# XuZerui2023/Radar-Signal-Process

Hardware: AMD Instinct MI355X
Metric: CPIs/sec (4096 range × 128 pulse) through PC→MTD→CFAR; achieved HBM GB/s (higher is better)
Workload: dtype f32

## Files before the change

include/rsp.h:

```cpp
#ifndef RSP_H
#define RSP_H

#include <stddef.h>
#include <stdint.h>

#ifdef __cplusplus
extern "C" {
#endif

#define RSP_ABI_VERSION 5
#define RSP_MAX_SEG 4
#define RSP_MAX_FIR_TAPS 64

typedef struct rsp_ctx rsp_ctx;

typedef enum {
    RSP_OK = 0,
    RSP_ERR_ARG = 1,
    RSP_ERR_SHAPE = 2,
    RSP_ERR_UNSUPPORTED = 3,
    RSP_ERR_CFAR_WINDOW = 4,
    RSP_ERR_HIP = 5,
    RSP_ERR_NOMEM = 6
} rsp_status;
// ... 98 lines not shown
int rsp_pc_mtd_cfar_f64(rsp_ctx* ctx, const void* echo, int32_t dtype, int32_t layout,
                        int64_t P, int64_t R, int64_t batch, const rsp_cfar_params* cfar,
                        double* rdm_out , int32_t out_layout, double* flag_out,
                        double* flagV_out );
int rsp_cfar_f64(rsp_ctx* ctx, const double* rdm, int32_t rdm_layout, int64_t V, int64_t R,
                 int64_t batch, const rsp_cfar_params* cfar, double* flag_out,
                 double* flagV_out );

int rsp_pc_mtd_cfar_dev(rsp_ctx* ctx, const void* d_echo, int32_t dtype, int64_t batch,
                        const rsp_cfar_params* cfar, float* d_rdm, uint8_t* d_flag,
                        uint8_t* d_flagV, void* stream);

int rsp_cfar_dev(rsp_ctx* ctx, const float* d_rdm, int64_t V, int64_t R, int64_t batch,
                 const rsp_cfar_params* cfar, uint8_t* d_flag, uint8_t* d_flagV,
                 void* stream);

int rsp_mtd_cfar_dev(rsp_ctx* ctx, const void* d_pc, int64_t batch, const rsp_cfar_params* cfar,
                     float* d_rdm, uint8_t* d_flag, uint8_t* d_flagV, void* stream);

int rsp_pc_mtd_cfar_diff_dev(rsp_ctx* ctx, const void* d_echo, int32_t dtype, int64_t batch,
                             const rsp_cfar_params* cfar, float* d_sum, float* d_diff,
                             uint8_t* d_flag, uint8_t* d_flagV, void* stream);

int rsp_window_pc_mtd_cfar_dev(rsp_ctx* ctx, const void* d_frames, int32_t dtype, int64_t beams,
                               int64_t frames, int32_t win, const rsp_cfar_params* cfar,
                               float* d_rdm, uint8_t* d_flag, uint8_t* d_flagV, void* stream);

int rsp_pc_dev(rsp_ctx* ctx, const void* d_echo, int32_t dtype, int64_t batch, void* d_pc,
               void* stream);

int rsp_set_pc_split(rsp_ctx* ctx, int32_t enable);

int rsp_set_pc_prune(rsp_ctx* ctx, int32_t enable);

typedef struct {
    int32_t nfft;
    int32_t nsub;
    int32_t sub_step;
    int32_t zin;
    int32_t zout;
    int32_t fir;
} rsp_pc_plan_seg;
typedef struct {
    int32_t specialised;
    int32_t fused;
    int32_t prune;
    int32_t nmf;
    rsp_pc_plan_seg seg[RSP_MAX_SEG];
} rsp_pc_plan_t;
int rsp_pc_plan(rsp_ctx* ctx, rsp_pc_plan_t* out, int32_t n);

enum { RSP_CFAR_R_COPY = 0,
       RSP_CFAR_R_GENERIC = 1,
       RSP_CFAR_R_4CELL = 2,
       RSP_CFAR_R_16CELL = 3 };
enum { RSP_RANGE_NONE = 0,
       RSP_RANGE_GROUPED = 1,
       RSP_RANGE_JOB57 = 2,
       RSP_RANGE_PREV_HITS = 3,
       RSP_RANGE_PER_CHUNK = 4 };
enum { RSP_HITS_NONE = 0,
       RSP_HITS_BATCHED57 = 1,
       RSP_HITS_PER_HIT57 = 2,
       RSP_HITS_PER_HIT_RUNTIME = 3 };
typedef struct {
    int32_t fused;
// ... 231 lines not shown
```

radar-signal-process_amd/csrc/rsp_capi.cpp:

```cpp
#include <hip/hip_runtime.h>

#include <cmath>
#include <complex>
#include <cstdarg>
#include <cstdio>
#include <cstdlib>
#include <cstring>
#include <map>
#include <new>
#include <string>
#include <vector>

#include "rsp_ctx.h"

using rsp::make_window;
using rsp::scratch_acquire;
using rsp::scratch_release;
using rsp::upload;

using cd = std::complex<double>;

static thread_local std::string g_err;

int fail(rsp_ctx* ctx, int code, const char* fmt, ...) {
    char buf[512];
    va_list ap;
    va_start(ap, fmt);
    vsnprintf(buf, sizeof(buf), fmt, ap);
    va_end(ap);
    if (ctx) ctx->err = buf;
    g_err = buf;
    return code;
}


static double mround(double x) { return x >= 0 ? std::floor(x + 0.5) : -std::floor(-x + 0.5); }

static double bessel_i0(double x) {
    double sum = 1.0, term = 1.0, q = x * x / 4.0;
    for (int k = 1; k < 500; ++k) {
        term *= q / ((double)k * k);
        sum += term;
        if (term < 1e-18 * sum) break;
    }
    return sum;
}
// ... 741 lines not shown
    if (!ctx) return fail(nullptr, RSP_ERR_ARG, "rsp_set_range_concat: null ctx");
    if (ctx->cfar_only) return fail(ctx, RSP_ERR_ARG, "rsp_set_range_concat: CFAR-only context");
    if (nparts < 0 || nparts > RSP_MAX_SEG || (nparts > 0 && (!src_start || !len)))
        return fail(ctx, RSP_ERR_ARG, "rsp_set_range_concat: bad part list (%d parts)", nparts);
    int64_t w = 0;
    for (int i = 0; i < nparts; ++i) {
        if (len[i] < 1 || src_start[i] < 0 || src_start[i] + len[i] > ctx->pc_w)
            return fail(ctx, RSP_ERR_ARG, "rsp_set_range_concat: part %d [%lld, +%lld) outside the %lld PC columns", i,
                        (long long)src_start[i], (long long)len[i], (long long)ctx->pc_w);
        w += len[i];
    }
    if (!set_device(ctx)) return fail(ctx, RSP_ERR_HIP, "hipSetDevice failed");
    HIP_TRY(ctx, hipDeviceSynchronize());
    ctx->ncat = nparts;
    for (int i = 0; i < nparts; ++i) {
        ctx->cat_src[i] = src_start[i];
        ctx->cat_len[i] = len[i];
    }
    ctx->p.R_out = nparts > 0 ? w : ctx->pc_w;
    ctx->mtd.R_out = (int)ctx->p.R_out;
    return RSP_OK;
}

static bool pc_fused(const rsp_ctx* ctx) {
    return ctx->pc_mf.size() == 2 && rsp::pc_pair_supported(ctx->pc_mf[0].mf.nfft, ctx->pc_mf[1].mf.nfft);
}
static rsp::PcMfArgs pc_launch_args(const rsp_ctx* ctx, size_t i, int64_t rows) {
    rsp::PcMfArgs a = ctx->pc_mf[i];
    a.rows = (int)rows;
    if (!ctx->pc_prune) a.zin = a.zout = 0;
    return a;
}

static hipError_t run_pc_rows(rsp_ctx* ctx, const void* ein, int dtype, float2* out, int64_t rows, hipStream_t s) {
    if (!ctx->pc_v2)
        return timed(ctx, RSP_K_PC, s, [&] { return rsp::launch_pc(ein, dtype, out, rows, ctx->pc, ctx->pc_lds, s); });
    if (pc_fused(ctx)) {
        const rsp::PcMfArgs a1 = pc_launch_args(ctx, 0, rows), a2 = pc_launch_args(ctx, 1, rows);
        return timed(ctx, RSP_K_PC, s, [&] { return rsp::launch_pc_mf(ein, dtype, out, a1, &a2, s); });
    }
    for (size_t i = 0; i < ctx->pc_mf.size(); ++i) {
        const rsp::PcMfArgs a = pc_launch_args(ctx, i, rows);
        hipError_t e = timed(ctx, RSP_K_PC, s, [&] { return rsp::launch_pc_mf(ein, dtype, out, a, nullptr, s); });
        if (e != hipSuccess) return e;
    }
    return hipSuccess;
}

int rsp_pc_plan(rsp_ctx* ctx, rsp_pc_plan_t* out, int32_t n) {
    if (!ctx || !out) return fail(ctx, RSP_ERR_ARG, "rsp_pc_plan: null argument");
    if (ctx->cfar_only) return fail(ctx, RSP_ERR_ARG, "rsp_pc_plan: CFAR-only context");
    if (n < 0 || n > RSP_MAX_SEG || (size_t)n < ctx->pc_mf.size())
        return fail(ctx, RSP_ERR_ARG, "rsp_pc_plan: room for %d segments, the context has %d", n, (int)ctx->pc_mf.size());
    std::memset(out, 0, sizeof(*out));
    out->specialised = ctx->pc_v2 ? 1 : 0;
    if (!ctx->pc_v2) return RSP_OK;
    out->nmf = (int32_t)ctx->pc_mf.size();
    out->fused = pc_fused(ctx) ? 1 : 0;
    for (size_t i = 0; i < ctx->pc_mf.size(); ++i) {
        const rsp::PcMfArgs a = pc_launch_args(ctx, i, 1);
        rsp_pc_plan_seg& g = out->seg[i];
        g.nfft = a.mf.nfft;
        g.nsub = a.nsub;
        g.sub_step = a.sub_step;
        g.zin = a.zin;
        g.zout = a.zout;
        g.fir = a.do_fir;
    }
    if (out->fused) {
        const rsp::PcMfArgs a1 = pc_launch_args(ctx, 0, 1), a2 = pc_launch_args(ctx, 1, 1);
        out->prune = rsp::pc_prune_select(a1, &a2);
    } else {
        for (size_t i = 0; i < ctx->pc_mf.size(); ++i) {
            const rsp::PcMfArgs a = pc_launch_args(ctx, i, 1);
            if (const int pr = rsp::pc_prune_select(a, nullptr)) out->prune = pr;
        }
// ... 45 lines not shown
    if (ctx->ncat == 0) {
        HIP_TRY(ctx, run_pc(ctx, d_echo, dtype, (float2*)d_pc, batch * ctx->p.P, (hipStream_t)stream, 0, 0));
        return RSP_OK;
    }
    hipStream_t s = (hipStream_t)stream;
    int rc = scratch_acquire(ctx, s);
    if (rc) return rc;
    if ((rc = cat_ensure(ctx, 1, batch * ctx->p.P))) return rc;
    HIP_TRY(ctx, run_pc(ctx, d_echo, dtype, (float2*)d_pc, batch * ctx->p.P, s, 0, batch * ctx->p.P));
    return scratch_release(ctx, s);
}

int rsp_set_pc_split(rsp_ctx* ctx, int32_t enable) {
    if (!ctx) return fail(nullptr, RSP_ERR_ARG, "rsp_set_pc_split: null ctx");
    if (ctx->cfar_only) return fail(ctx, RSP_ERR_ARG, "rsp_set_pc_split: CFAR-only context");
    if (!ctx->pc_v2)
        return fail(ctx, RSP_ERR_UNSUPPORTED, "rsp_set_pc_split: this context has no specialised PC path");
    const std::vector<rsp::PcMfArgs>& src = enable ? ctx->pc_mf_split : ctx->pc_mf_whole;
    for (size_t i = 0; i < ctx->pc_mf.size() && i < src.size(); ++i) {
        const float* gain = ctx->pc_mf[i].gain;
        ctx->pc_mf[i] = src[i];
        ctx->pc_mf[i].gain = gain;
    }
    return RSP_OK;
}

int rsp_set_pc_prune(rsp_ctx* ctx, int32_t enable) {
    if (!ctx) return fail(nullptr, RSP_ERR_ARG, "rsp_set_pc_prune: null ctx");
    if (ctx->cfar_only) return fail(ctx, RSP_ERR_ARG, "rsp_set_pc_prune: CFAR-only context");
    if (!ctx->pc_v2)
        return fail(ctx, RSP_ERR_UNSUPPORTED, "rsp_set_pc_prune: this context has no specialised PC path");
    ctx->pc_prune = enable != 0;
    return RSP_OK;
}

int rsp_set_prefilter(rsp_ctx* ctx, const float* gain, int32_t mti_lag) {
    if (!ctx) return fail(nullptr, RSP_ERR_ARG, "rsp_set_prefilter: null ctx");
    if (ctx->cfar_only) return fail(ctx, RSP_ERR_ARG, "rsp_set_prefilter: CFAR-only context");
    if (mti_lag < 0) return fail(ctx, RSP_ERR_ARG, "rsp_set_prefilter: negative MTI lag %d", mti_lag);
    if (gain && !ctx->pc_v2)
        return fail(ctx, RSP_ERR_UNSUPPORTED, "rsp_set_prefilter: the fused gain needs the per-segment PC kernels");
    if (!set_device(ctx)) return fail(ctx, RSP_ERR_HIP, "hipSetDevice failed");
    HIP_TRY(ctx, hipDeviceSynchronize());
    const float* d_gain = nullptr;
    if (gain) {
        const size_t bytes = (size_t)ctx->p.R * sizeof(float);
        const int rc = ensure(ctx, ctx->pf_gain, bytes);
        if (rc) return rc;
        HIP_TRY(ctx, hipMemcpy(ctx->pf_gain.p, gain, bytes, hipMemcpyHostToDevice));
        d_gain = (const float*)ctx->pf_gain.p;
    }
    for (rsp::PcMfArgs& a : ctx->pc_mf) a.gain = d_gain;
    ctx->mtd.mti_lag = mti_lag;
    return RSP_OK;
}

static constexpr int kRangeGroup = 16;
static constexpr uint64_t kRangeGroupBytes = 1ull << 30;
static int range_mode() {
    static const int m = [] { const char* v = getenv("RSP_RANGE_MODE"); return v && *v ? atoi(v) : 2; }();
    return m;
}
static int range_group() {
    static const int g = [] { const char* v = getenv("RSP_RANGE_GROUP"); const int x = v && *v ? atoi(v) : kRangeGroup; return x < 1 ? 1 : x; }();
    return g;
}
// ... 412 lines not shown
```

radar-signal-process_amd/csrc/rsp_ctx.h:

```cpp
#pragma once
#include <hip/hip_runtime.h>

#include <cstdint>
#include <cstdlib>
#include <map>
#include <memory>
#include <string>
#include <vector>

#include "../../include/rsp.h"
#include "rsp_hostpool.h"
#include "rsp_chunkplan.h"
#include "rsp_hostplan.h"
#include "rsp_internal.h"

struct DevBuf {
    void* p = nullptr;
    size_t n = 0;
};

struct rsp_ctx {
    int device = 0;
    bool cfar_only = false;
    rsp_params p{};
    std::string err;
    hipStream_t stream = nullptr;
    rsp::PcArgs pc{};
    bool pc_v2 = false;
#ifndef RSP_PC_OLS_MIN
#define RSP_PC_OLS_MIN 4096
#endif
    int pc_ols_min = RSP_PC_OLS_MIN;
    std::vector<rsp::PcMfArgs> pc_mf_whole, pc_mf_split;
    std::vector<rsp::PcMfArgs> pc_mf;
    int64_t lane_cpis[rsp::kMaxLanes] = {};
    int nlane_cpis = 0;
    bool pc_prune = [] { const char* v = getenv("RSP_PC_PRUNE"); return !(v && *v == '0'); }();
    rsp::MtdArgs mtd{};
    int64_t V = 0;
    int beams = 1;
    size_t pc_lds = 0;
    int64_t chunk = 0;
    int nstreams = 0;
    hipStream_t aux[3] = {nullptr, nullptr, nullptr};
    hipEvent_t ev_fork = nullptr, ev_join[3] = {nullptr, nullptr, nullptr};
    hipEvent_t ev_scratch = nullptr;
    bool scratch_pending = false;
    std::vector<void*> owned;
    std::map<int, float2*> tw;
    DevBuf scratch_pc, tmp_flagV, tmp_rdm;
    int64_t pc_w = 0;
    int ncat = 0;
    int64_t cat_src[RSP_MAX_SEG] = {}, cat_len[RSP_MAX_SEG] = {};
    DevBuf cat_tmp;
    DevBuf pf_gain;
    DevBuf hit_list;
    DevBuf hit_ctr;
    DevBuf meas_band;
    DevBuf scr_ps;
    DevBuf cond_tmp;
    DevBuf cmap_band;
    std::map<std::vector<int64_t>, float2*> cmap_tab;
    DevBuf ing_meta;
    DevBuf st_in, st_canon, st_rdm, st_flag, st_flagV, st_t;
    struct HostPipe {
        static constexpr int kSlots = 2;
        static constexpr int kRing = 4;
        hipStream_t s_h2d = nullptr, s_d2h = nullptr;
        DevBuf in[kSlots], canon[kSlots], rdm[kSlots], flag[kSlots], flagV[kSlots], tr[kSlots][3];
        hipEvent_t ev_in[kSlots] = {}, ev_comp[kSlots] = {}, ev_out[kSlots] = {};
// ... 57 lines not shown
```

radar-signal-process_amd/csrc/rsp_internal.h:

```cpp
#pragma once
#include <hip/hip_runtime.h>
#include <math.h>
#include <stdint.h>

#include <mutex>

#include "../../include/rsp.h"

namespace rsp {

constexpr int kBlock = 256;

constexpr int kMaxDevices = 64;
struct LaunchOnce {
    std::once_flag once[kMaxDevices];
    hipError_t err[kMaxDevices] = {};
    int value[kMaxDevices] = {};
};
template <typename F>
inline hipError_t launch_once(LaunchOnce& L, int* value, F&& init) {
    int dev = 0;
    hipError_t e = hipGetDevice(&dev);
    if (e != hipSuccess) return e;
    if (dev < 0 || dev >= kMaxDevices) return hipErrorInvalidDevice;
// ... 255 lines not shown
struct LegacyIngestArgs {
    int prt_num, point_prt, nframes;
    int64_t rows;
    int64_t rows_decoded;
    int64_t rec_bytes, nbytes;
    int64_t beam_stride, frame_stride;
};
hipError_t launch_ingest_legacy(const uint8_t* stream, const LegacyIngestArgs& a, float2* out, double* angle,
                                int32_t* head, int32_t* status, hipStream_t s);

constexpr int64_t ingest_payload_bytes(uint32_t type, int64_t pdn, int64_t ch) {
    const int64_t sig = type == 0 ? pdn * ch * 2
                      : type == 1 ? pdn * ch * 4
                                  : pdn * ch * 6 + pdn * (8 - (6 * ch) % 8);
    return sig % 64 ? sig + 64 - sig % 64 : sig;
}
constexpr int dbf24_row_bytes(int ch) { return 6 * ch + (8 - (6 * ch) % 8); }
constexpr int dbf24_values(int ch) {
    const int L = dbf24_row_bytes(ch);
    const int n1 = L - 3 >= 1 ? (L - 4) / 3 + 1 : 0, n2 = L - 2 >= 2 ? (L - 4) / 3 + 1 : 0, n3 = L / 3;
    return (n1 == n2 && n2 == n3 && n1 % 2 == 0) ? n1 : -1;
}

bool mtd_size_supported(int P, int beams = 1);
bool pc_nfft_supported(int n);
size_t pc_lds_bytes(int max_nfft);

hipError_t launch_pc(const void* echo, int dtype, float2* out, int64_t rows, const PcArgs& a,
                     size_t lds_bytes, hipStream_t s);
inline int fir_stage_len(const SegDev& g) { return g.ntaps4 - 1 + g.out_len + 4; }
bool pc_mf_supported(int nfft, int fir_stage_len);
bool pc_pair_supported(int nfft1, int nfft2);
int pc_prune_select(const PcMfArgs& a1, const PcMfArgs* a2);
hipError_t launch_pc_mf(const void* echo, int dtype, float2* out, const PcMfArgs& a1, const PcMfArgs* a2,
                        hipStream_t s);
hipError_t launch_mtd(const float2* pc, float* rdm, uint8_t* flagV, int ncpi, const MtdArgs& a,
                      hipStream_t s);
hipError_t launch_cfar_v(const float* rdm, uint8_t* flagV, int ncpi, int V, int R,
                         const CfarVArgs& a, hipStream_t s);
hipError_t launch_cfar_hits(const float* rdm, uint8_t* flag, const uint32_t* hits, const uint32_t* counts,
                            int nregions, int region, const CfarRArgs& a, hipStream_t s);
int cfar_hits_select(const CfarRArgs& a, int nregions, int region, int* lpr);
int cfar_r_select(const CfarRArgs& a, int* groups);
int cfar_v_tile_log2(int V);
bool mtd_window_compiled(const MtdArgs& a);
bool mtd_range_job57(const MtdArgs& a);
bool mtd_geometry(int P, int beams, int* W, int* T);
void mtd_regions(int P, int R_out, int ncpi, int* nregions, int* region, int beams = 1);
int mtd_bluestein_nf(int P);
hipError_t launch_cfar_r(const float* rdm, const uint8_t* flagV, uint8_t* flag, int ncpi,
                         const CfarRArgs& a, hipStream_t s);
bool cfar_r_supported(const CfarRArgs& a);
hipError_t launch_canon(const void* in, int dtype, int layout, float2* out, int64_t batch,
                        int P, int R, hipStream_t s);
hipError_t launch_transpose_f32(const float* in, float* out, int64_t batch, int A, int B,
                                hipStream_t s);
hipError_t launch_transpose_u8(const uint8_t* in, uint8_t* out, int64_t batch, int A, int B,
                               hipStream_t s);
enum { RSP_SUB_F32 = 0, RSP_SUB_U8 = 1, RSP_SUB_C64 = 2, RSP_SUB_C32F16 = 3 };
hipError_t launch_transpose_sub(int elem, const void* in, void* out, int A, int B, size_t in_pitch, size_t out_pitch,
                                hipStream_t s);
hipError_t launch_copy_words(const void* in, void* out, size_t nwords, hipStream_t s);

}
```

radar-signal-process_amd/csrc/rsp_pc.hip:

```cpp
#include <hip/hip_fp16.h>
#include <hip/hip_runtime.h>

#include "rsp_fft.h"
#include "rsp_buf.h"
#include "rsp_diag.h"
#include "rsp_internal.h"

namespace rsp {

template <int N, typename TIn>
__device__ __forceinline__ void mf_segment(const TIn* __restrict__ x, float2* __restrict__ y,
                                           const SegDev& g, float2* lds, int t) {
    for (int i = t; i < N; i += kBlock) {
        float2 v = make_float2(0.f, 0.f);
        if (i < g.in_len) v = ld_c(x + g.in_start + i);
        lds[pidx(i)] = v;
    }
    __syncthreads();
    fft_lds<N, kBlock>(lds, t, g.tw);
    for (int i = t; i < N; i += kBlock) lds[pidx(i)] = cconj(cmul(lds[pidx(i)], g.H[i]));
    __syncthreads();
    fft_lds<N, kBlock>(lds, t, g.tw);
    for (int i = t; i < g.out_len; i += kBlock) y[g.out_start + i] = cconj(lds[pidx(i)]);
    __syncthreads();
}

template <typename TIn>
__device__ __forceinline__ void fir_segment(const TIn* __restrict__ x, float2* __restrict__ y,
                                            const SegDev& g, int t) {
    const int len = g.out_len;
    for (int n = t; n < len; n += kBlock) {
        int m = n + g.fir_shift;
        m %= len;
        float ar = 0.f, ai = 0.f;
#pragma unroll 8
        for (int k = 0; k < RSP_MAX_FIR_TAPS; ++k) {
            if (k < g.ntaps && k <= m) {
                const float2 v = ld_c(x + g.in_start + m - k);
                ar = fmaf(g.taps[k], v.x, ar);
// ... 274 lines not shown
            cmul2_conj(u[m], u[m], hs[m], u[m + 1], u[m + 1], hs[m + 1]);
    } else {
        constexpr int HB = 8;
#pragma unroll
        for (int m0 = 0; m0 < E; m0 += HB) {
            float2 h[HB];
#pragma unroll
            for (int m = 0; m < HB; ++m) h[m] = buf_ld_f2(hr, (uint32_t)e0 * 8u, (uint32_t)(G * (m0 + m)) * 8u);
#pragma unroll
            for (int m = 0; m < HB; m += 2)
                cmul2_conj(u[m0 + m], u[m0 + m], h[m], u[m0 + m + 1], u[m0 + m + 1], h[m + 1]);
        }
    }
    RSP_STAMP(0, 4, false);
    if constexpr (!kDiagPcNoFft) fft_reg_w<N, G, 1, E, 0, NW, WS, 0, ZOUT>(u, buf, t, w);
    RSP_STAMP(0, 5, false);
    if constexpr (kUniform) {
        const auto yr = buf_rsrc(y + out_start, st_ok ? (uint32_t)out_len * 8u : 0u);
#pragma unroll
        for (int m = 0; m < EO; ++m) buf_st_f2(cconj(u[m]), yr, (uint32_t)e0 * 8u, (uint32_t)(G * m) * 8u);
    } else if (st_ok) {
#pragma unroll
        for (int m = 0; m < E; ++m) {
            const int i = t + G * m;
            if (i < out_len) *(y + out_start + i) = cconj(u[m]);
        }
    }
    RSP_STAMP(0, 6, false);
    RSP_STAMP(0, 7, true);
    RSP_STAMP_RT(0, 9);
}


template <int N1, int N2>
struct PairCfg {
    static constexpr int T0 = PcCfg<N1>::G > PcCfg<N2>::G ? PcCfg<N1>::G : PcCfg<N2>::G;
    static constexpr int T = T0 < 256 ? 256 : T0;
    static constexpr int RPB1 = T / PcCfg<N1>::G, RPB2 = T / PcCfg<N2>::G;
    static constexpr size_t L1 = (size_t)RPB1 * PcCfg<N1>::SLOT * sizeof(float2);
    static constexpr size_t L2 = (size_t)RPB2 * PcCfg<N2>::SLOT * sizeof(float2);
    static constexpr size_t lds = L1 > L2 ? L1 : L2;
};

constexpr int pc_prune_code(int zi1, int zo1, int zi2, int zo2) { return zi1 << 12 | zo1 << 8 | zi2 << 4 | zo2; }
template <typename TIn, int N1, int N2, int PR = 0>
__device__ __forceinline__ void pc_mf_block(const TIn* __restrict__ echo, float2* __restrict__ out, const PcMfArgs& a1,
                                            const PcMfArgs& a2, int nblk2, int bid, float2* lds) {
    constexpr int M2 = N2 ? N2 : N1;
    using PC = PairCfg<N1, M2>;
    if constexpr (N2 != 0) {
        if (bid < nblk2) {
            constexpr int G = PcCfg<N2>::G;
            const int grp = threadIdx.x / G, t = threadIdx.x % G;
            const int ns = a2.nsub > 1 ? a2.nsub : 1;
            const int u = bid * PC::RPB2 + grp;
            pc_row<TIn, N2, G, G == 64, (PR >> 4 & 15), (PR & 15)>(echo, out, a2, u / ns, t,
                                                                   lds + grp * PcCfg<N2>::SLOT, u % ns);
            return;
        }
    }
    constexpr int G = PcCfg<N1>::G;
    const int grp = threadIdx.x / G, t = threadIdx.x % G;
    const int b = bid - (N2 ? nblk2 : 0);
    const int u = b * PC::RPB1 + grp, ns = a1.nsub > 1 ? a1.nsub : 1;
    pc_row<TIn, N1, G, G == 64, (PR >> 12 & 15), (PR >> 8 & 15)>(echo, out, a1, u / ns, t,
                                                                 lds + grp * PcCfg<N1>::SLOT, u % ns);
}

template <typename TIn, int N1, int N2, int PR = 0>
__global__ __launch_bounds__((PairCfg<N1, (N2 ? N2 : N1)>::T), RSP_DIAG_PC_WAVES) void pc_mf_kernel(
    const TIn* __restrict__ echo, float2* __restrict__ out, PcMfArgs a1, PcMfArgs a2, int nblk2) {
    extern __shared__ __attribute__((aligned(16))) float2 lds[];
    RSP_STAMP(0, 0, false);
    RSP_STAMP_RT(0, 8);
    pc_mf_block<TIn, N1, N2, PR>(echo, out, a1, a2, nblk2, (int)blockIdx.x, lds);
}


bool pc_mf_supported(int nfft, int fir_stage_len) {
    switch (nfft) {
        case 64: case 128: case 256: case 512: case 1024: case 2048: case 4096: case 8192:
        case 16384:
            return fir_stage_len <= padded_len(nfft);
        default:
            return false;
    }
}

template <typename TIn, int N1, int N2, int PR = 0>
static hipError_t launch_pc_mf_n(const TIn* echo, float2* out, const PcMfArgs& a1, const PcMfArgs* a2,
                                 hipStream_t s) {
    constexpr int M2 = N2 ? N2 : N1;
    using PC = PairCfg<N1, M2>;
    static LaunchOnce once;
    constexpr size_t lds = PC::lds + kDiagPcLdsExtra;
    hipError_t e = lds_attr(once, (const void*)pc_mf_kernel<TIn, N1, N2, PR>, lds);
    if (e != hipSuccess) return e;
    const int u1 = a1.rows * (a1.nsub > 1 ? a1.nsub : 1);
    const int nblk1 = (u1 + PC::RPB1 - 1) / PC::RPB1;
    const int u2 = a2 ? a2->rows * (a2->nsub > 1 ? a2->nsub : 1) : 0;
    const int nblk2 = N2 ? (u2 + PC::RPB2 - 1) / PC::RPB2 : 0;
    dim3 grid((unsigned)(nblk1 + nblk2)), block(PC::T);
    hipLaunchKernelGGL((pc_mf_kernel<TIn, N1, N2, PR>), grid, block, lds, s, echo, out, a1, a2 ? *a2 : a1, nblk2);
    return hipGetLastError();
}

#define RSP_PAIR(n1, n2) \
    if (a1.mf.nfft == n1 && a2 && a2->mf.nfft == n2) return launch_pc_mf_n<TIn, n1, n2>(echo, out, a1, a2, s)

int pc_prune_select(const PcMfArgs& a1, const PcMfArgs* a2) {
    if (a1.mf.nfft == 1024 && a2 && a2->mf.nfft == 4096 && a1.zin >= 4 && a1.zout >= 4) {
        if (a2->zin >= 3 && a2->zout >= 3) return pc_prune_code(4, 4, 3, 3);
        if (a2->zout >= 2) return pc_prune_code(4, 4, 0, 2);
    }
    return 0;
}

template <typename TIn>
static hipError_t launch_pc_mf_t(const TIn* echo, float2* out, const PcMfArgs& a1, const PcMfArgs* a2,
                                 hipStream_t s) {
    switch (pc_prune_select(a1, a2)) {
        case pc_prune_code(4, 4, 3, 3):
            return launch_pc_mf_n<TIn, 1024, 4096, pc_prune_code(4, 4, 3, 3)>(echo, out, a1, a2, s);
        case pc_prune_code(4, 4, 0, 2):
            return launch_pc_mf_n<TIn, 1024, 4096, pc_prune_code(4, 4, 0, 2)>(echo, out, a1, a2, s);
        default: break;
    }
    RSP_PAIR(1024, 1024);
    RSP_PAIR(1024, 4096);
    RSP_PAIR(1024, 8192);
    RSP_PAIR(1024, 16384);
    RSP_PAIR(512, 1024);
    if (a2) return hipErrorNotSupported;
    switch (a1.mf.nfft) {
        case 64: return launch_pc_mf_n<TIn, 64, 0>(echo, out, a1, nullptr, s);
        case 128: return launch_pc_mf_n<TIn, 128, 0>(echo, out, a1, nullptr, s);
        case 256: return launch_pc_mf_n<TIn, 256, 0>(echo, out, a1, nullptr, s);
        case 512: return launch_pc_mf_n<TIn, 512, 0>(echo, out, a1, nullptr, s);
        case 1024: return launch_pc_mf_n<TIn, 1024, 0>(echo, out, a1, nullptr, s);
        case 2048: return launch_pc_mf_n<TIn, 2048, 0>(echo, out, a1, nullptr, s);
        case 4096: return launch_pc_mf_n<TIn, 4096, 0>(echo, out, a1, nullptr, s);
        case 8192: return launch_pc_mf_n<TIn, 8192, 0>(echo, out, a1, nullptr, s);
        case 16384: return launch_pc_mf_n<TIn, 16384, 0>(echo, out, a1, nullptr, s);
        default: return hipErrorInvalidValue;
    }
}
#undef RSP_PAIR

#ifdef RSP_DIAG_STAMPS
}
extern "C" int rsp_diag_stamps(int k, uint64_t* host, int64_t n) {
    if (k < 0 || k > 1) return -1;
    return k == 0 ? rsp::diag_fetch(host, n) : rsp::diag_fetch_mtd(host, n);
}
namespace rsp {
#endif

bool pc_pair_supported(int n1, int n2) {
    return (n1 == 1024 && (n2 == 1024 || n2 == 4096 || n2 == 8192 || n2 == 16384)) || (n1 == 512 && n2 == 1024);
}

hipError_t launch_pc_mf(const void* echo, int dtype, float2* out, const PcMfArgs& a1, const PcMfArgs* a2,
                        hipStream_t s) {
    if (a1.rows <= 0) return hipSuccess;
    if (dtype == RSP_C64) return launch_pc_mf_t((const float2*)echo, out, a1, a2, s);
    if (dtype == RSP_C32F16) return launch_pc_mf_t((const __half2*)echo, out, a1, a2, s);
    return hipErrorInvalidValue;
}

}
```

radar-signal-process_amd/rsp/_capi.py:

```python
import ctypes as C
import os

_HERE = os.path.dirname(os.path.abspath(__file__))
LIB_PATH = os.path.join(os.path.dirname(_HERE), "lib", "librsp.so")

RSP_MAX_SEG = 4
RSP_MAX_FIR_TAPS = 64

RSP_OK, RSP_ERR_ARG, RSP_ERR_SHAPE, RSP_ERR_UNSUPPORTED, RSP_ERR_CFAR_WINDOW, RSP_ERR_HIP, RSP_ERR_NOMEM = range(7)
RSP_C64, RSP_C128, RSP_C32F16 = 0, 1, 2
RSP_ROWMAJOR, RSP_COLMAJOR = 0, 1
RSP_SEG_FIR, RSP_SEG_MF = 0, 1
RSP_WIN_KAISER, RSP_WIN_HAMMING, RSP_WIN_RECT = 0, 1, 2

EXPORTS = ("rsp_version", "rsp_create", "rsp_destroy", "rsp_last_error", "rsp_set_chunk",
           "rsp_pc_mtd", "rsp_cfar", "rsp_pc_mtd_cfar", "rsp_pc_mtd_cfar_dev", "rsp_cfar_dev",
           "rsp_pc_dev", "rsp_profile", "rsp_profile_read", "rsp_profile_read_n", "rsp_set_streams",
           "rsp_create_v2", "rsp_create_legacy", "rsp_window_pc_mtd_cfar_dev", "rsp_pc_mtd_cfar_diff_dev",
           "rsp_mtd_cfar_dev", "rsp_set_pc_split", "rsp_set_host_pipeline", "rsp_ingest_record_bytes",
           "rsp_ingest_ddc_dev", "rsp_ingest_frame_dev", "rsp_motion_measure_dev", "rsp_prefilter_dev", "rsp_set_prefilter",
           "rsp_pc_mtd_cfar_f64", "rsp_cfar_f64", "rsp_set_range_concat", "rsp_score_dev", "rsp_score_summary",
           "rsp_set_pc_prune", "rsp_set_lane_chunks", "rsp_pc_plan", "rsp_scr_dev", "rsp_inject_dev", "rsp_scr_gain",
           "rsp_cfar_plan", "rsp_legacy_record_bytes", "rsp_ingest_legacy_dev", "rsp_condense_dev", "rsp_cmap_dev",
           "rsp_cmap_plan", "rsp_spec_width_dev", "rsp_track_dev")
RSP_NKERNELS = 4
KERNEL_NAMES = ("pc_kernel", "mtd_kernel", "cfar_r_kernel", "cfar_v_kernel")


class RspError(RuntimeError):
    def __init__(self, code, msg):
        super().__init__("rsp error %d: %s" % (code, msg))
        self.code = code


class rsp_pc_segment(C.Structure):
    _fields_ = [("kind", C.c_int32), ("fir_shift", C.c_int32),
                ("in_start", C.c_int64), ("in_len", C.c_int64),
                ("out_start", C.c_int64), ("out_len", C.c_int64),
                ("nfft", C.c_int64), ("scale", C.c_double),
                ("coef_len", C.c_int64),
                ("coef_re", C.POINTER(C.c_double)), ("coef_im", C.POINTER(C.c_double))]


class rsp_params(C.Structure):
    _fields_ = [("P", C.c_int64), ("R", C.c_int64), ("R_out", C.c_int64),
                ("nseg", C.c_int32), ("window", C.c_int32), ("window_beta", C.c_double),
                ("fftshift", C.c_int32), ("zero_v_div", C.c_int32),
                ("seg", rsp_pc_segment * RSP_MAX_SEG),
                ("mtd_nfft", C.c_int64), ("beams", C.c_int32), ("zero_ends", C.c_int32)]


class rsp_cfar_params(C.Structure):
    _fields_ = [("refR", C.c_int32), ("saveR", C.c_int32), ("methodR", C.c_int32), ("TR", C.c_double),
                ("refV", C.c_int32), ("saveV", C.c_int32), ("methodV", C.c_int32), ("TV", C.c_double),
                ("M0", C.c_int32), ("rFlag", C.c_int32), ("zero_v_div", C.c_int32),
                ("nseg", C.c_int32),
                ("seg_lo", C.c_int64 * RSP_MAX_SEG), ("seg_hi", C.c_int64 * RSP_MAX_SEG)]
# ... 137 lines not shown
    lib.rsp_pc_mtd_cfar.restype = C.c_int
    lib.rsp_pc_mtd_cfar.argtypes = [vp, vp, i32, i32, i64, i64, i64, C.POINTER(rsp_cfar_params),
                                    vp, i32, vp, vp]
    lib.rsp_pc_mtd_cfar_f64.restype = C.c_int
    lib.rsp_pc_mtd_cfar_f64.argtypes = [vp, vp, i32, i32, i64, i64, i64, C.POINTER(rsp_cfar_params),
                                        vp, i32, vp, vp]
    lib.rsp_cfar_f64.restype = C.c_int
    lib.rsp_cfar_f64.argtypes = [vp, vp, i32, i64, i64, i64, C.POINTER(rsp_cfar_params), vp, vp]
    lib.rsp_pc_mtd_cfar_dev.restype = C.c_int
    lib.rsp_pc_mtd_cfar_dev.argtypes = [vp, vp, i32, i64, C.POINTER(rsp_cfar_params), vp, vp, vp, vp]
    lib.rsp_cfar_dev.restype = C.c_int
    lib.rsp_cfar_dev.argtypes = [vp, vp, i64, i64, i64, C.POINTER(rsp_cfar_params), vp, vp, vp]
    lib.rsp_window_pc_mtd_cfar_dev.restype = C.c_int
    lib.rsp_window_pc_mtd_cfar_dev.argtypes = [vp, vp, i32, i64, i64, i32, C.POINTER(rsp_cfar_params), vp, vp, vp,
                                               vp]
    lib.rsp_pc_mtd_cfar_diff_dev.restype = C.c_int
    lib.rsp_pc_mtd_cfar_diff_dev.argtypes = [vp, vp, i32, i64, C.POINTER(rsp_cfar_params), vp, vp, vp, vp, vp]
    lib.rsp_mtd_cfar_dev.restype = C.c_int
    lib.rsp_mtd_cfar_dev.argtypes = [vp, vp, i64, C.POINTER(rsp_cfar_params), vp, vp, vp, vp]
    lib.rsp_pc_dev.restype = C.c_int
    lib.rsp_pc_dev.argtypes = [vp, vp, i32, i64, vp, vp]
    lib.rsp_create_v2.restype = C.c_int
    lib.rsp_create_v2.argtypes = [C.POINTER(vp), C.c_int, i64, i64, C.POINTER(i64), C.c_double, C.c_double,
                                  C.POINTER(C.c_double)]
    dp = C.POINTER(C.c_double)
    lib.rsp_create_legacy.restype = C.c_int
    lib.rsp_create_legacy.argtypes = [C.POINTER(vp), C.c_int, i64, i64, dp, dp, i64, dp, dp, i64]
    lib.rsp_set_streams.restype = C.c_int
    lib.rsp_set_streams.argtypes = [vp, i32]
    lib.rsp_set_pc_split.restype = C.c_int
    lib.rsp_set_pc_split.argtypes = [vp, i32]
    lib.rsp_set_pc_prune.restype = C.c_int
    lib.rsp_set_pc_prune.argtypes = [vp, i32]
    lib.rsp_pc_plan.restype = C.c_int
    lib.rsp_pc_plan.argtypes = [vp, C.POINTER(rsp_pc_plan_t), i32]
    lib.rsp_cfar_plan.restype = C.c_int
    lib.rsp_cfar_plan.argtypes = [vp, i64, i64, i64, C.POINTER(rsp_cfar_params), i32, i32, C.POINTER(rsp_cfar_plan_t)]
    lib.rsp_set_lane_chunks.restype = C.c_int
    lib.rsp_set_lane_chunks.argtypes = [vp, C.POINTER(i64), i32]
    lib.rsp_set_host_pipeline.restype = C.c_int
    lib.rsp_set_host_pipeline.argtypes = [vp, i64, i32]
    lib.rsp_set_prefilter.restype = C.c_int
    lib.rsp_set_prefilter.argtypes = [vp, C.POINTER(C.c_float), i32]
    lib.rsp_ingest_record_bytes.restype = C.c_int
    lib.rsp_ingest_record_bytes.argtypes = [C.POINTER(rsp_ingest_params), C.POINTER(i64)]
    lib.rsp_ingest_ddc_dev.restype = C.c_int
    lib.rsp_ingest_ddc_dev.argtypes = [vp, vp, i64, C.POINTER(rsp_ingest_params), vp, vp, i64, vp, vp, vp]
    lib.rsp_ingest_frame_dev.restype = C.c_int
    lib.rsp_ingest_frame_dev.argtypes = [vp, vp, i64, C.POINTER(rsp_ingest_params), vp, vp, i64, vp, vp, vp]
    lib.rsp_legacy_record_bytes.restype = C.c_int
    lib.rsp_legacy_record_bytes.argtypes = [C.POINTER(rsp_legacy_ingest_params), C.POINTER(i64)]
    lib.rsp_ingest_legacy_dev.restype = C.c_int
    lib.rsp_ingest_legacy_dev.argtypes = [vp, vp, i64, C.POINTER(rsp_legacy_ingest_params), vp, i64, i64, vp, vp, vp, vp]
    lib.rsp_motion_measure_dev.restype = C.c_int
    lib.rsp_motion_measure_dev.argtypes = [vp, vp, vp, vp, i64, i64, i64, C.POINTER(rsp_measure_params), vp, vp,
                                           i64, vp, vp, vp, vp]
    lib.rsp_condense_dev.restype = C.c_int
    lib.rsp_condense_dev.argtypes = [vp, vp, vp, i64, i64, i64, C.POINTER(rsp_condense_params), vp, i32, vp, vp, vp]
    lib.rsp_cmap_dev.restype = C.c_int
    lib.rsp_cmap_dev.argtypes = [vp, vp, i64, i64, C.POINTER(rsp_cmap_params), vp, i32, vp, vp, vp, vp, vp]
    lib.rsp_cmap_plan.restype = C.c_int
    lib.rsp_cmap_plan.argtypes = [vp, i64, i64, C.POINTER(rsp_cmap_params), C.POINTER(rsp_cmap_plan_t)]
    lib.rsp_spec_width_dev.restype = C.c_int
    lib.rsp_spec_width_dev.argtypes = [vp, vp, vp, i64, i64, i64, C.POINTER(rsp_width_params), vp, vp, vp]
    lib.rsp_track_dev.restype = C.c_int
    lib.rsp_track_dev.argtypes = [vp, vp, vp, i64, i64, C.POINTER(rsp_track_params), vp, vp, i32, vp, vp, vp, vp, vp,
# ... 34 lines not shown
```

radar-signal-process_amd/rsp/engine.py:

```python
import ctypes as C

import numpy as np

from . import _capi as capi
from . import presets


def _ptr(a):
    return C.c_void_p(a.ctypes.data) if a is not None else None


class Engine:
    def __init__(self, spec, device=0, chunk=0, streams=0):
        self.spec = spec
        self.lib = capi.load_library()
        ctx = C.c_void_p()
        if spec is None:
            rc = self.lib.rsp_create(C.byref(ctx), int(device), None)
        else:
            prm, self._keep = spec.to_c()
            rc = self.lib.rsp_create(C.byref(ctx), int(device), C.byref(prm))
        capi.check(rc, None)
        self.ctx = ctx
        self.device = device
# ... 13 lines not shown
        try:
            self.close()
        except Exception:
            pass

    def __enter__(self):
        return self

    def __exit__(self, *exc):
        self.close()

    def set_streams(self, n):
        capi.check(self.lib.rsp_set_streams(self.ctx, int(n)), self.ctx)

    def set_range_concat(self, parts):
        n = len(parts)
        src = (C.c_int64 * max(n, 1))(*[int(a) for a, _ in parts])
        ln = (C.c_int64 * max(n, 1))(*[int(b) for _, b in parts])
        capi.check(self.lib.rsp_set_range_concat(self.ctx, n, src, ln), self.ctx)

    def set_chunk(self, cpis):
        capi.check(self.lib.rsp_set_chunk(self.ctx, int(cpis)), self.ctx)

    def set_lane_chunks(self, cpis=()):
        n = len(cpis)
        arr = (C.c_int64 * max(n, 1))(*[int(c) for c in cpis])
        capi.check(self.lib.rsp_set_lane_chunks(self.ctx, arr, n), self.ctx)

    def set_pc_split(self, enable):
        capi.check(self.lib.rsp_set_pc_split(self.ctx, int(enable)), self.ctx)

    def set_pc_prune(self, enable):
        capi.check(self.lib.rsp_set_pc_prune(self.ctx, int(enable)), self.ctx)

    def pc_plan(self):
        p = capi.rsp_pc_plan_t()
        capi.check(self.lib.rsp_pc_plan(self.ctx, C.byref(p), capi.RSP_MAX_SEG), self.ctx)
        segs = [(g.nfft, g.nsub, g.sub_step, g.zin, g.zout, g.fir) for g in p.seg[:p.nmf]]
        return dict(specialised=p.specialised, fused=p.fused, prune=p.prune, segs=segs)

    def cfar_plan(self, cfar, batch, V=None, R=None, fused=None, rdm=True):
        if fused is None:
            fused = self.spec is not None
        if fused:
            V, R = self.spec.V, self.spec.R_out
        p = capi.rsp_cfar_plan_t()
        cp = cfar.to_c()
        capi.check(self.lib.rsp_cfar_plan(self.ctx, int(V), int(R), int(batch), C.byref(cp), int(bool(fused)),
                                          int(bool(rdm)), C.byref(p)), self.ctx)
        if not fused:
            return dict(fused=0, v_tile_log2=p.v_tile_log2, r_kernel=p.r_kernel, r_groups=p.r_groups)
        n = p.nlanes
        return dict(fused=1, window_compiled=p.window_compiled, bluestein=p.bluestein, tile_w=p.tile_w,
                    threads=p.threads, region=p.region, nchunks=p.nchunks, nlanes=n,
                    lane_chunk=list(p.lane_chunk[:n]), lane_last=list(p.lane_last[:n]), range_stage=p.range_stage,
                    hit_kernel=p.hit_kernel, hit_lanes=p.hit_lanes, flag_memset=p.flag_memset)

    def set_host_pipeline(self, cpis_per_chunk=0, copy_threads=0):
        capi.check(self.lib.rsp_set_host_pipeline(self.ctx, int(cpis_per_chunk), int(copy_threads)), self.ctx)

    def set_prefilter(self, gain=None, mti_lag=0):
        g = None
        if gain is not None:
            g = np.ascontiguousarray(gain, dtype=np.float32)
            if g.shape != (self.spec.R,):
                raise ValueError("gain must have R = %d entries" % self.spec.R)
# ... 199 lines not shown
```

Measured before the change: 311,100.

## Process multiple rows per PC workgroup to reuse twiddles and filter spectrum

Adds a multi-row pulse-compression path for 4096-point FFTs in which each workgroup group loops over 2 or 4 rows. The twiddle registers and matched-filter spectrum are loaded once and reused across those rows, and the grid shrinks to match. The default is 2 rows, settable through an environment variable or a new API. The aim is to amortise the per-row setup loads and launch overhead, at the cost of fewer workgroups, less parallelism and more template instantiations.

After: 315,300, median of 6. 1.3% higher.

```diff
diff --git a/include/rsp.h b/include/rsp.h
--- a/include/rsp.h
+++ b/include/rsp.h
@@ -154,6 +154,9 @@
 int rsp_set_pc_split(rsp_ctx* ctx, int32_t enable);
 
 int rsp_set_pc_prune(rsp_ctx* ctx, int32_t enable);
+
+int rsp_set_pc_rows(rsp_ctx* ctx, int32_t n);
+int rsp_get_pc_rows(rsp_ctx* ctx);
 
 typedef struct {
     int32_t nfft;
diff --git a/radar-signal-process_amd/csrc/rsp_capi.cpp b/radar-signal-process_amd/csrc/rsp_capi.cpp
--- a/radar-signal-process_amd/csrc/rsp_capi.cpp
+++ b/radar-signal-process_amd/csrc/rsp_capi.cpp
@@ -12,6 +12,7 @@
 #include <vector>
 
 #include "rsp_ctx.h"
+#include "rsp_pcplan.h"
 
 using rsp::make_window;
 using rsp::scratch_acquire;
@@ -819,16 +820,26 @@
     return a;
 }
 
+static int pc_rows_want(const rsp_ctx* ctx) {
+    static const int dflt = [] {
+        const char* v = getenv("RSP_PC_ROWS");
+        const int n = v ? atoi(v) : 0;
+        return rsp::pc_rows_valid(n) ? n : rsp::kPcRowsDefault;
+    }();
+    return ctx->pc_rows ? ctx->pc_rows : dflt;
+}
+
 static hipError_t run_pc_rows(rsp_ctx* ctx, const void* ein, int dtype, float2* out, int64_t rows, hipStream_t s) {
+    const int want = ctx->pc_v2 ? pc_rows_want(ctx) : 1;
     if (!ctx->pc_v2)
         return timed(ctx, RSP_K_PC, s, [&] { return rsp::launch_pc(ein, dtype, out, rows, ctx->pc, ctx->pc_lds, s); });
     if (pc_fused(ctx)) {
         const rsp::PcMfArgs a1 = pc_launch_args(ctx, 0, rows), a2 = pc_launch_args(ctx, 1, rows);
-        return timed(ctx, RSP_K_PC, s, [&] { return rsp::launch_pc_mf(ein, dtype, out, a1, &a2, s); });
+        return timed(ctx, RSP_K_PC, s, [&] { return rsp::launch_pc_mf(ein, dtype, out, a1, &a2, want, s); });
     }
     for (size_t i = 0; i < ctx->pc_mf.size(); ++i) {
         const rsp::PcMfArgs a = pc_launch_args(ctx, i, rows);
-        hipError_t e = timed(ctx, RSP_K_PC, s, [&] { return rsp::launch_pc_mf(ein, dtype, out, a, nullptr, s); });
+        hipError_t e = timed(ctx, RSP_K_PC, s, [&] { return rsp::launch_pc_mf(ein, dtype, out, a, nullptr, want, s); });
         if (e != hipSuccess) return e;
     }
     return hipSuccess;
@@ -940,6 +951,32 @@
         return fail(ctx, RSP_ERR_UNSUPPORTED, "rsp_set_pc_prune: this context has no specialised PC path");
     ctx->pc_prune = enable != 0;
     return RSP_OK;
+}
+
+int rsp_set_pc_rows(rsp_ctx* ctx, int32_t n) {
+    if (!ctx) return fail(nullptr, RSP_ERR_ARG, "rsp_set_pc_rows: null ctx");
+    if (ctx->cfar_only) return fail(ctx, RSP_ERR_ARG, "rsp_set_pc_rows: CFAR-only context");
+    if (!ctx->pc_v2)
+        return fail(ctx, RSP_ERR_UNSUPPORTED, "rsp_set_pc_rows: this context has no specialised PC path");
+    if (n != 0 && !rsp::pc_rows_valid(n)) return fail(ctx, RSP_ERR_ARG, "rsp_set_pc_rows: %d is not 0, 1, 2 or 4", (int)n);
+    ctx->pc_rows = n;
+    return RSP_OK;
+}
+
+int rsp_get_pc_rows(rsp_ctx* ctx) {
+    if (!ctx || ctx->cfar_only || !ctx->pc_v2) return 1;
+    const int want = pc_rows_want(ctx);
+    if (pc_fused(ctx)) {
+        const rsp::PcMfArgs a1 = pc_launch_args(ctx, 0, 1), a2 = pc_launch_args(ctx, 1, 1);
+        return rsp::pc_rows_select(a1, &a2, want);
+    }
+    int rows = 1;
+    for (size_t i = 0; i < ctx->pc_mf.size(); ++i) {
+        const rsp::PcMfArgs a = pc_launch_args(ctx, i, 1);
+        const int r = rsp::pc_rows_select(a, nullptr, want);
+        if (r > rows) rows = r;
+    }
+    return rows;
 }
 
 int rsp_set_prefilter(rsp_ctx* ctx, const float* gain, int32_t mti_lag) {
diff --git a/radar-signal-process_amd/csrc/rsp_ctx.h b/radar-signal-process_amd/csrc/rsp_ctx.h
--- a/radar-signal-process_amd/csrc/rsp_ctx.h
+++ b/radar-signal-process_amd/csrc/rsp_ctx.h
@@ -36,6 +36,7 @@
     int64_t lane_cpis[rsp::kMaxLanes] = {};
     int nlane_cpis = 0;
     bool pc_prune = [] { const char* v = getenv("RSP_PC_PRUNE"); return !(v && *v == '0'); }();
+    int pc_rows = 0;
     rsp::MtdArgs mtd{};
     int64_t V = 0;
     int beams = 1;
diff --git a/radar-signal-process_amd/csrc/rsp_internal.h b/radar-signal-process_amd/csrc/rsp_internal.h
--- a/radar-signal-process_amd/csrc/rsp_internal.h
+++ b/radar-signal-process_amd/csrc/rsp_internal.h
@@ -311,8 +311,9 @@
 bool pc_mf_supported(int nfft, int fir_stage_len);
 bool pc_pair_supported(int nfft1, int nfft2);
 int pc_prune_select(const PcMfArgs& a1, const PcMfArgs* a2);
+int pc_rows_select(const PcMfArgs& a1, const PcMfArgs* a2, int want);
 hipError_t launch_pc_mf(const void* echo, int dtype, float2* out, const PcMfArgs& a1, const PcMfArgs* a2,
-                        hipStream_t s);
+                        int pc_rows, hipStream_t s);
 hipError_t launch_mtd(const float2* pc, float* rdm, uint8_t* flagV, int ncpi, const MtdArgs& a,
                       hipStream_t s);
 hipError_t launch_cfar_v(const float* rdm, uint8_t* flagV, int ncpi, int V, int R,
diff --git a/radar-signal-process_amd/csrc/rsp_pc.hip b/radar-signal-process_amd/csrc/rsp_pc.hip
--- a/radar-signal-process_amd/csrc/rsp_pc.hip
+++ b/radar-signal-process_amd/csrc/rsp_pc.hip
@@ -5,6 +5,7 @@
 #include "rsp_buf.h"
 #include "rsp_diag.h"
 #include "rsp_internal.h"
+#include "rsp_pcplan.h"
 
 namespace rsp {
 
@@ -345,6 +346,70 @@
 }
 
 
+template <typename TIn, int N, int G, int ROWS, int ZIN = 0, int ZOUT = 0>
+__device__ __forceinline__ void pc_rows(const TIn* __restrict__ echo, float2* __restrict__ out,
+                                        const PcMfArgs& a, int u0, int t, float2* buf) {
+    constexpr int E = N / G;
+    static_assert(G % 64 == 0 && G > 64, "rows of whole waves, exchanged through the workgroup barrier");
+    static_assert(N <= 4096, "the spectrum slice stays in registers");
+    static_assert(ZIN >= 0 && ZIN < E && ZOUT >= 0 && ZOUT < E, "a row keeps at least one slice");
+    constexpr int EI = E - ZIN, EO = E - ZOUT;
+    constexpr uint32_t ES = sizeof(TIn);
+    const int e0 = t;
+    const float2* __restrict__ tw = a.mf.tw;
+    const auto hr = buf_rsrc(a.mf.H, (uint32_t)N * 8u);
+    constexpr int NW = tw_regs<N, E>() > 0 ? tw_regs<N, E>() : 1;
+    float2 w[NW];
+    tw_preload<N, G, 1, E, 0, NW>(w, t, tw);
+    float2 hs[E];
+#pragma unroll
+    for (int m = 0; m < E; ++m) hs[m] = buf_ld_f2(hr, (uint32_t)e0 * 8u, (uint32_t)(G * m) * 8u);
+    const int ns = a.nsub > 1 ? a.nsub : 1;
+#pragma unroll 1
+    for (int k = 0; k < ROWS; ++k) {
+        const int unit = __builtin_amdgcn_readfirstlane(u0 + k);
+        const int row = __builtin_amdgcn_readfirstlane(unit / ns);
+        const int sub = __builtin_amdgcn_readfirstlane(unit % ns);
+        const bool valid = row < a.rows;
+        const TIn* x = echo + (size_t)diag_pc_src_row(row) * a.R;
+        const bool st_ok = valid && !kDiagPcNoStore;
+        float2* y = out + (size_t)row * a.R_out;
+        int in_start = a.mf.in_start, in_len = a.mf.in_len;
+        int out_start = a.mf.out_start, out_len = a.mf.out_len;
+        if (a.nsub > 1) {
+            const int off = sub * a.sub_step;
+            in_start = __builtin_amdgcn_readfirstlane(in_start + off);
+            out_start = __builtin_amdgcn_readfirstlane(out_start + off);
+            in_len = __builtin_amdgcn_readfirstlane(max(0, min(in_len - off, N)));
+            out_len = __builtin_amdgcn_readfirstlane(max(0, min(out_len - off, a.sub_step)));
+        }
+        float2 u[E];
+        const auto xr = buf_rsrc(x + in_start, valid ? (uint32_t)in_len * ES : 0u);
+#pragma unroll
+        for (int m = 0; m < EI; ++m) u[m] = buf_ld_c((const TIn*)nullptr, xr, (uint32_t)e0 * ES, (uint32_t)(G * m) * ES);
+#pragma unroll
+        for (int m = EI; m < E; ++m) u[m] = make_float2(0.f, 0.f);
+        if (a.gain) {
+            const auto gr = buf_rsrc(a.gain + in_start, (uint32_t)in_len * 4u);
+#pragma unroll
+            for (int m = 0; m < EI; ++m) u[m] = cscale(u[m], buf_ld_f(gr, (uint32_t)e0 * 4u, (uint32_t)(G * m) * 4u));
+        }
+        if (a.nzero > 0 && valid && sub == 0) {
+            for (int z = 0; z < a.nzero; ++z)
+                for (int c = a.zero_lo[z] + t; c < a.zero_hi[z]; c += G) y[c] = make_float2(0.f, 0.f);
+        }
+        if constexpr (!kDiagPcNoFft) fft_reg_w<N, G, 1, E, 0, NW, false, ZIN, 0>(u, buf, t, w);
+#pragma unroll
+        for (int m = 0; m < E; m += 2)
+            cmul2_conj(u[m], u[m], hs[m], u[m + 1], u[m + 1], hs[m + 1]);
+        if constexpr (!kDiagPcNoFft) fft_reg_w<N, G, 1, E, 0, NW, false, 0, ZOUT>(u, buf, t, w);
+        const auto yr = buf_rsrc(y + out_start, st_ok ? (uint32_t)out_len * 8u : 0u);
+#pragma unroll
+        for (int m = 0; m < EO; ++m) buf_st_f2(cconj(u[m]), yr, (uint32_t)e0 * 8u, (uint32_t)(G * m) * 8u);
+    }
+}
+
+
 template <int N1, int N2>
 struct PairCfg {
     static constexpr int T0 = PcCfg<N1>::G > PcCfg<N2>::G ? PcCfg<N1>::G : PcCfg<N2>::G;
@@ -355,8 +420,9 @@
     static constexpr size_t lds = L1 > L2 ? L1 : L2;
 };
 
+constexpr bool pc_rows_built(int n, int rows) { return rows == 1 || (n == 4096 && (rows == 2 || rows == 4)); }
 constexpr int pc_prune_code(int zi1, int zo1, int zi2, int zo2) { return zi1 << 12 | zo1 << 8 | zi2 << 4 | zo2; }
-template <typename TIn, int N1, int N2, int PR = 0>
+template <typename TIn, int N1, int N2, int PR = 0, int ROWS = 1>
 __device__ __forceinline__ void pc_mf_block(const TIn* __restrict__ echo, float2* __restrict__ out, const PcMfArgs& a1,
                                             const PcMfArgs& a2, int nblk2, int bid, float2* lds) {
     constexpr int M2 = N2 ? N2 : N1;
@@ -367,8 +433,14 @@
             const int grp = threadIdx.x / G, t = threadIdx.x % G;
             const int ns = a2.nsub > 1 ? a2.nsub : 1;
             const int u = bid * PC::RPB2 + grp;
-            pc_row<TIn, N2, G, G == 64, (PR >> 4 & 15), (PR & 15)>(echo, out, a2, u / ns, t,
-                                                                   lds + grp * PcCfg<N2>::SLOT, u % ns);
+            if constexpr (ROWS > 1) {
+                static_assert(pc_rows_built(N2, ROWS), "no multi-row path for this length");
+                pc_rows<TIn, N2, G, ROWS, (PR >> 4 & 15), (PR & 15)>(echo, out, a2, u * ROWS, t,
+                                                                     lds + grp * PcCfg<N2>::SLOT);
+            } else {
+                pc_row<TIn, N2, G, G == 64, (PR >> 4 & 15), (PR & 15)>(echo, out, a2, u / ns, t,
+                                                                       lds + grp * PcCfg<N2>::SLOT, u % ns);
+            }
             return;
         }
     }
@@ -376,17 +448,23 @@
     const int grp = threadIdx.x / G, t = threadIdx.x % G;
     const int b = bid - (N2 ? nblk2 : 0);
     const int u = b * PC::RPB1 + grp, ns = a1.nsub > 1 ? a1.nsub : 1;
-    pc_row<TIn, N1, G, G == 64, (PR >> 12 & 15), (PR >> 8 & 15)>(echo, out, a1, u / ns, t,
-                                                                 lds + grp * PcCfg<N1>::SLOT, u % ns);
-}
-
-template <typename TIn, int N1, int N2, int PR = 0>
+    if constexpr (N2 == 0 && ROWS > 1) {
+        static_assert(pc_rows_built(N1, ROWS), "no multi-row path for this length");
+        pc_rows<TIn, N1, G, ROWS, (PR >> 12 & 15), (PR >> 8 & 15)>(echo, out, a1, u * ROWS, t,
+                                                                   lds + grp * PcCfg<N1>::SLOT);
+    } else {
+        pc_row<TIn, N1, G, G == 64, (PR >> 12 & 15), (PR >> 8 & 15)>(echo, out, a1, u / ns, t,
+                                                                     lds + grp * PcCfg<N1>::SLOT, u % ns);
+    }
+}
+
+template <typename TIn, int N1, int N2, int PR = 0, int ROWS = 1>
 __global__ __launch_bounds__((PairCfg<N1, (N2 ? N2 : N1)>::T), RSP_DIAG_PC_WAVES) void pc_mf_kernel(
     const TIn* __restrict__ echo, float2* __restrict__ out, PcMfArgs a1, PcMfArgs a2, int nblk2) {
     extern __shared__ __attribute__((aligned(16))) float2 lds[];
     RSP_STAMP(0, 0, false);
     RSP_STAMP_RT(0, 8);
-    pc_mf_block<TIn, N1, N2, PR>(echo, out, a1, a2, nblk2, (int)blockIdx.x, lds);
+    pc_mf_block<TIn, N1, N2, PR, ROWS>(echo, out, a1, a2, nblk2, (int)blockIdx.x, lds);
 }
 
 
@@ -400,21 +478,21 @@
     }
 }
 
-template <typename TIn, int N1, int N2, int PR = 0>
+template <typename TIn, int N1, int N2, int PR = 0, int ROWS = 1>
 static hipError_t launch_pc_mf_n(const TIn* echo, float2* out, const PcMfArgs& a1, const PcMfArgs* a2,
                                  hipStream_t s) {
     constexpr int M2 = N2 ? N2 : N1;
     using PC = PairCfg<N1, M2>;
     static LaunchOnce once;
     constexpr size_t lds = PC::lds + kDiagPcLdsExtra;
-    hipError_t e = lds_attr(once, (const void*)pc_mf_kernel<TIn, N1, N2, PR>, lds);
+    hipError_t e = lds_attr(once, (const void*)pc_mf_kernel<TIn, N1, N2, PR, ROWS>, lds);
     if (e != hipSuccess) return e;
     const int u1 = a1.rows * (a1.nsub > 1 ? a1.nsub : 1);
-    const int nblk1 = (u1 + PC::RPB1 - 1) / PC::RPB1;
+    const int nblk1 = pc_blocks(u1, PC::RPB1, N2 ? 1 : ROWS);
     const int u2 = a2 ? a2->rows * (a2->nsub > 1 ? a2->nsub : 1) : 0;
-    const int nblk2 = N2 ? (u2 + PC::RPB2 - 1) / PC::RPB2 : 0;
+    const int nblk2 = N2 ? pc_blocks(u2, PC::RPB2, ROWS) : 0;
     dim3 grid((unsigned)(nblk1 + nblk2)), block(PC::T);
-    hipLaunchKernelGGL((pc_mf_kernel<TIn, N1, N2, PR>), grid, block, lds, s, echo, out, a1, a2 ? *a2 : a1, nblk2);
+    hipLaunchKernelGGL((pc_mf_kernel<TIn, N1, N2, PR, ROWS>), grid, block, lds, s, echo, out, a1, a2 ? *a2 : a1, nblk2);
     return hipGetLastError();
 }
 
@@ -429,15 +507,36 @@
     return 0;
 }
 
+int pc_rows_select(const PcMfArgs& a1, const PcMfArgs* a2, int want) {
+    if (!pc_rows_valid(want) || want == 1) return 1;
+    if (a2) return a1.mf.nfft == 1024 && a2->mf.nfft == 4096 && !a2->do_fir ? want : 1;
+    return a1.mf.nfft == 4096 && !a1.do_fir ? want : 1;
+}
+
+template <typename TIn, int N1, int N2, int PR>
+static hipError_t launch_pc_mf_r(const TIn* echo, float2* out, const PcMfArgs& a1, const PcMfArgs* a2, int rows,
+                                 hipStream_t s) {
+    switch (rows) {
+        case 4: return launch_pc_mf_n<TIn, N1, N2, PR, 4>(echo, out, a1, a2, s);
+        case 2: return launch_pc_mf_n<TIn, N1, N2, PR, 2>(echo, out, a1, a2, s);
+        default: return launch_pc_mf_n<TIn, N1, N2, PR, 1>(echo, out, a1, a2, s);
+    }
+}
+
 template <typename TIn>
-static hipError_t launch_pc_mf_t(const TIn* echo, float2* out, const PcMfArgs& a1, const PcMfArgs* a2,
+static hipError_t launch_pc_mf_t(const TIn* echo, float2* out, const PcMfArgs& a1, const PcMfArgs* a2, int want,
                                  hipStream_t s) {
+    const int rows = pc_rows_select(a1, a2, want);
     switch (pc_prune_select(a1, a2)) {
         case pc_prune_code(4, 4, 3, 3):
-            return launch_pc_mf_n<TIn, 1024, 4096, pc_prune_code(4, 4, 3, 3)>(echo, out, a1, a2, s);
+            return launch_pc_mf_r<TIn, 1024, 4096, pc_prune_code(4, 4, 3, 3)>(echo, out, a1, a2, rows, s);
         case pc_prune_code(4, 4, 0, 2):
-            return launch_pc_mf_n<TIn, 1024, 4096, pc_prune_code(4, 4, 0, 2)>(echo, out, a1, a2, s);
+            return launch_pc_mf_r<TIn, 1024, 4096, pc_prune_code(4, 4, 0, 2)>(echo, out, a1, a2, rows, s);
         default: break;
+    }
+    if (rows > 1) {
+        if (a2) return launch_pc_mf_r<TIn, 1024, 4096, 0>(echo, out, a1, a2, rows, s);
+        return launch_pc_mf_r<TIn, 4096, 0, 0>(echo, out, a1, nullptr, rows, s);
     }
     RSP_PAIR(1024, 1024);
     RSP_PAIR(1024, 4096);
@@ -474,10 +573,10 @@
 }
 
 hipError_t launch_pc_mf(const void* echo, int dtype, float2* out, const PcMfArgs& a1, const PcMfArgs* a2,
-                        hipStream_t s) {
+                        int pc_rows, hipStream_t s) {
     if (a1.rows <= 0) return hipSuccess;
-    if (dtype == RSP_C64) return launch_pc_mf_t((const float2*)echo, out, a1, a2, s);
-    if (dtype == RSP_C32F16) return launch_pc_mf_t((const __half2*)echo, out, a1, a2, s);
+    if (dtype == RSP_C64) return launch_pc_mf_t((const float2*)echo, out, a1, a2, pc_rows, s);
+    if (dtype == RSP_C32F16) return launch_pc_mf_t((const __half2*)echo, out, a1, a2, pc_rows, s);
     return hipErrorInvalidValue;
 }
 
diff --git a/radar-signal-process_amd/csrc/rsp_pcplan.h b/radar-signal-process_amd/csrc/rsp_pcplan.h
--- /dev/null
+++ b/radar-signal-process_amd/csrc/rsp_pcplan.h
@@ -0,0 +1,16 @@
+#pragma once
+#include <cstdint>
+
+namespace rsp {
+
+constexpr int kPcRowsDefault = 2;
+
+inline bool pc_rows_valid(int n) { return n == 1 || n == 2 || n == 4; }
+
+inline int pc_blocks(int64_t units, int rpb, int rows) {
+    if (units <= 0 || rpb < 1 || rows < 1) return 0;
+    const int64_t per = (int64_t)rpb * rows;
+    return (int)((units + per - 1) / per);
+}
+
+}
diff --git a/radar-signal-process_amd/rsp/_capi.py b/radar-signal-process_amd/rsp/_capi.py
--- a/radar-signal-process_amd/rsp/_capi.py
+++ b/radar-signal-process_amd/rsp/_capi.py
@@ -22,7 +22,7 @@
            "rsp_pc_mtd_cfar_f64", "rsp_cfar_f64", "rsp_set_range_concat", "rsp_score_dev", "rsp_score_summary",
            "rsp_set_pc_prune", "rsp_set_lane_chunks", "rsp_pc_plan", "rsp_scr_dev", "rsp_inject_dev", "rsp_scr_gain",
            "rsp_cfar_plan", "rsp_legacy_record_bytes", "rsp_ingest_legacy_dev", "rsp_condense_dev", "rsp_cmap_dev",
-           "rsp_cmap_plan", "rsp_spec_width_dev", "rsp_track_dev")
+           "rsp_cmap_plan", "rsp_spec_width_dev", "rsp_track_dev", "rsp_set_pc_rows", "rsp_get_pc_rows")
 RSP_NKERNELS = 4
 KERNEL_NAMES = ("pc_kernel", "mtd_kernel", "cfar_r_kernel", "cfar_v_kernel")
 
@@ -226,6 +226,10 @@
     lib.rsp_set_pc_split.argtypes = [vp, i32]
     lib.rsp_set_pc_prune.restype = C.c_int
     lib.rsp_set_pc_prune.argtypes = [vp, i32]
+    lib.rsp_set_pc_rows.restype = C.c_int
+    lib.rsp_set_pc_rows.argtypes = [vp, i32]
+    lib.rsp_get_pc_rows.restype = C.c_int
+    lib.rsp_get_pc_rows.argtypes = [vp]
     lib.rsp_pc_plan.restype = C.c_int
     lib.rsp_pc_plan.argtypes = [vp, C.POINTER(rsp_pc_plan_t), i32]
     lib.rsp_cfar_plan.restype = C.c_int
diff --git a/radar-signal-process_amd/rsp/engine.py b/radar-signal-process_amd/rsp/engine.py
--- a/radar-signal-process_amd/rsp/engine.py
+++ b/radar-signal-process_amd/rsp/engine.py
@@ -69,6 +69,12 @@
 
     def set_pc_prune(self, enable):
         capi.check(self.lib.rsp_set_pc_prune(self.ctx, int(enable)), self.ctx)
+
+    def set_pc_rows(self, n):
+        capi.check(self.lib.rsp_set_pc_rows(self.ctx, int(n)), self.ctx)
+
+    def pc_rows(self):
+        return int(self.lib.rsp_get_pc_rows(self.ctx))
 
     def pc_plan(self):
         p = capi.rsp_pc_plan_t()
```
